# ROAM-Lab-ND/generalized_rbda

Measured on AMD Instinct MI355X. Metric: forward-dynamics evals/sec (batched random states), MIT Humanoid cluster model, higher is better.
Workload: dtype f32; 1 GPU; mit_humanoid.urdf cluster-ABA, 262144 random states per GPU; batch_per_gpu=262144, batch_global=262144, nq=25, nv=24, n_bodies=37, n_clusters=17, parallelism=batch-sharded x1, plan replicated

## Files before the change

generalized_rbda_amd/csrc/capi.cpp:

```cpp
#include <hip/hip_runtime.h>

#include <array>
#include <cassert>
#include <cmath>
#include <cstdio>
#include <cstdlib>
#include <cstring>
#include <map>
#include <memory>
#include <mutex>
#include <string>
#include <vector>

#include "../../include/grbda_hip.h"
#include "../../include/grbda_hip_vjp.h"
#include "../../include/grbda_hip_step_vjp.h"
#include "../../include/grbda_hip_jvp.h"
#include "../../include/grbda_hip_wrench.h"
#include "../../include/grbda_hip_bodies.h"
#include "../../include/grbda_hip_jacobians.h"
#include "../../include/grbda_model_desc.h"
#include "devplan.h"

namespace grbda_hip {
// ... 573 lines not shown
template <class T>
int run_chain(const grbda_plan *p, const DeviceTables &t, const Route &r, const T *q, const T *qd, const T *tau, T *ydd, size_t B, int device,
              void *stream, bool gravity = true, const WrenchList<T> *wrenches = nullptr)
{
    const HostPlan &h = p->host;
    const ChainProgram &cp = h.chain[r.slot];
    const size_t n_tiles = (B + kWave - 1) / kWave;
    const size_t in_rows = static_cast<size_t>(h.nq + 2 * h.nv);
    const hipStream_t hs = static_cast<hipStream_t>(stream);
    ChainDev<T> d = chain_dev<T>(p, t, r.slot);
    if (!gravity)
        for (int i = 0; i < 6; i++) d.a_root[i] = T(0);
    void *scratch = nullptr;
    if (r.path == ROUTE_GEN1) {
        gen1_only(d);
        d.sv_global = 0;
        d.out_lds = -1;
        d.lds_bytes = static_cast<int>(static_cast<size_t>(cp.n_lds) * kWave * sizeof(T));
        const size_t lds_total = gen1_lds_bytes<T>(h, cp);
        const size_t grid = gen1_grid(p, t.n_cu, n_tiles, gen1_waves_per_simd<T>(cp.gens[0].n), lds_total);
        hipError_t e = launch_aba_gen1<T>(d, cp.gens[0].n, cp.gens[0].kind != 0, q, qd, tau, ydd, B, static_cast<int>(grid), lds_total, hs);
        return e == hipSuccess ? GRBDA_OK : hip_err(e, "aba single-cluster launch");
    }
    if (r.path == ROUTE_LM) {
        if (cp.diffs.empty()) d.diffs = nullptr;
        no_gens(d);
        d.n_glb_slots = cp.n_glb + 1;
        d.sv_global = 0;
        const size_t lds_lm = lm_lds_bytes<T>(h, cp);
        d.lds_bytes = static_cast<int>(lds_lm);
        const size_t grid = n_tiles;
        if (int rc = ensure_scratch(p, device, stream, scratch_bytes(grid, static_cast<size_t>(d.n_glb_slots) + in_rows, sizeof(T)), &scratch)) return rc;
        hipError_t e = launch_aba_chain_lm<T>(d, q, qd, tau, ydd, B, static_cast<T *>(scratch), static_cast<int>(grid), lds_lm, hs, r.lm_waves);
        return e == hipSuccess ? GRBDA_OK : hip_err(e, "aba chain launch (latency mode)");
    }
    const int kid = sizeof(T) == 8 ? 1 : 0;
    const size_t waves_per_cu = static_cast<size_t>((sizeof(T) == 8 && !cp.gens.empty()) ? p->opt.waves_per_cu_f64_wide_regs : p->opt.waves_per_cu[kid]);
    const LaunchShape s = launch_shape(t.n_cu, n_tiles, waves_per_cu, static_cast<size_t>(cp.n_lds) * kWave * sizeof(T), h.nq, h.nv, sizeof(T),
                                       static_cast<size_t>(p->opt.lds_bytes_per_wave[kid]), true);
    {
        int n_free_bwd = 0, at_bwd = -1;
        for (size_t i = 0; i < cp.segs.size(); i++)
            if (cp.segs[i].op == SEG_FREE_BWD) { n_free_bwd++; at_bwd = static_cast<int>(i); }
        if (!cp.segs.empty() && cp.segs[0].op == SEG_FREE_FWD && n_free_bwd == 1 && cp.frees[cp.segs[0].first].lds_v >= 0) {
            if (s.stage_all_fits) d.fuse |= 1;
            d.stage_lds_v = cp.frees[cp.segs[0].first].lds_v;
            d.stage_v_index = cp.frees[cp.segs[0].first].v_index;
        }
        if (n_free_bwd == 1 && at_bwd + 1 < static_cast<int>(cp.segs.size()) && cp.segs[at_bwd + 1].op == SEG_FREE_ACC &&
            cp.segs[at_bwd + 1].first == cp.segs[at_bwd].first)
            d.fuse |= 2;
    }
    d.lds_bytes = static_cast<int>(s.lds_bytes);
    if (int rc = ensure_scratch(p, device, stream, scratch_bytes(s.grid, static_cast<size_t>(cp.n_glb) + in_rows, sizeof(T)), &scratch)) return rc;
    hipError_t e = wrenches ? launch_aba_chain_wrench<T>(d, *wrenches, q, qd, tau, ydd, B, static_cast<T *>(scratch), static_cast<int>(s.grid), s.lds_bytes, hs)
                            : launch_aba_chain<T>(d, q, qd, tau, ydd, B, static_cast<T *>(scratch), static_cast<int>(s.grid), s.lds_bytes, hs);
    return e == hipSuccess ? GRBDA_OK : hip_err(e, "aba chain launch");
}

template <class T>
int run_rnea_chain(const grbda_plan *p, const DeviceTables &t, const Route &r, const T *q, const T *qd, const T *ydd, T *tau, size_t B, int device,
                   void *stream, bool gravity = true, const WrenchList<T> *wrenches = nullptr)
{
    const HostPlan &h = p->host;
    const RneaChainProgram &rp = h.rchain[r.slot];
    const size_t n_tiles = (B + kWave - 1) / kWave;
    const size_t in_rows = static_cast<size_t>(h.nq + 2 * h.nv);
    const hipStream_t hs = static_cast<hipStream_t>(stream);
    RneaChainDev<T> d = rnea_chain_dev<T>(p, t, r.slot);
    if (!gravity)
        for (int i = 0; i < 6; i++) d.a_root[i] = T(0);
    void *scratch = nullptr;
    if (r.path == ROUTE_LM) {
        if (rp.diffs.empty()) d.diffs = nullptr;
        no_gens(d);
        d.n_glb_slots = 0;
        const size_t lds_bytes = lm_lds_bytes<T>(h, rp);
        d.lds_bytes = static_cast<int>(lds_bytes);
        const size_t grid = n_tiles;
        if (int rc = ensure_scratch(p, device, stream, scratch_bytes(grid, in_rows, sizeof(T)), &scratch)) return rc;
        hipError_t e = launch_rnea_chain_lm<T>(d, q, qd, ydd, tau, B, static_cast<T *>(scratch), static_cast<int>(grid), lds_bytes, hs, r.lm_waves);
        return e == hipSuccess ? GRBDA_OK : hip_err(e, "rnea chain launch (latency mode)");
    }
    if (r.path == ROUTE_GEN1) {
        gen1_only(d);
        d.lds_bytes = static_cast<int>(static_cast<size_t>(rp.n_lds) * kWave * sizeof(T));
        const size_t lds_total = gen1_lds_bytes<T>(h, rp);
        const size_t grid = gen1_grid(p, t.n_cu, n_tiles, rnea_gen1_waves_per_simd<T>(rp.gens[0].n), lds_total);
        hipError_t e = launch_rnea_gen1<T>(d, rp.gens[0].n, rp.gens[0].kind != 0, q, qd, ydd, tau, B, static_cast<int>(grid), lds_total, hs);
        return e == hipSuccess ? GRBDA_OK : hip_err(e, "rnea single-cluster launch");
    }
    const bool wide = r.slot == SLOT_F32_WIDE;
    const int kid = sizeof(T) == 8 ? 1 : 0;
    const LaunchShape s = launch_shape(t.n_cu, n_tiles, wide ? static_cast<size_t>(16) : static_cast<size_t>(p->opt.waves_per_cu[kid]),
                                       static_cast<size_t>(rp.n_lds) * kWave * sizeof(T), h.nq, h.nv, sizeof(T),
                                       static_cast<size_t>(wide ? p->opt.chain32w_lds_bytes : p->opt.lds_bytes_per_wave[kid]), true);
    d.lds_bytes = static_cast<int>(s.lds_bytes);
    if (int rc = ensure_scratch(p, device, stream, scratch_bytes(s.grid, in_rows + static_cast<size_t>(rp.n_glb), sizeof(T)), &scratch)) return rc;
    const std::vector<ChainFree> &bases = h.chain[r.slot].frees;
    hipError_t e = wrenches ? launch_rnea_chain_wrench<T>(d, *wrenches, bases.empty() ? -1 : bases[0].body, q, qd, ydd, tau, B, static_cast<T *>(scratch),
                                                          static_cast<int>(s.grid), s.lds_bytes, hs)
                            : launch_rnea_chain<T>(d, q, qd, ydd, tau, B, static_cast<T *>(scratch), static_cast<int>(s.grid), s.lds_bytes, hs);
    return e == hipSuccess ? GRBDA_OK : hip_err(e, "rnea chain launch");
}

template <class T>
int projection_run(const grbda_plan *p, bool rnea, const T *q, const T *qd, const T *x, const T *f_ext, T *out, size_t B, int device, void *stream);
// ... 3896 lines not shown
```

generalized_rbda_amd/csrc/chain_kernels.hip:

```cpp
#include <hip/hip_runtime.h>

#include "devplan.h"

#ifndef GRBDA_CHAIN_UNIT
#define GRBDA_CHAIN_UNIT 0
#endif
#define GRBDA_KLDS (GRBDA_CHAIN_UNIT == 3)

namespace grbda_hip {

#include "devmath.h"

template <class T>
struct ChainTables {
    cptr<ChainSeg> segs;
    cptr<ChainLink> links;
    cptr<ChainPair> pairs;
    cptr<ChainFree> frees;
    cptr<ChainDiff> diffs;
    cptr<ChainGen> gens;
    cptr<ChainGenBody> gbodies;
    cptr<int32_t> cints;
    cptr<T> consts;
    int n_segs, nq, nv, ori_repr;
// ... 1461 lines not shown
    P.gens = (cptr<ChainGen>)DP.gens;
    P.gbodies = (cptr<ChainGenBody>)DP.gbodies;
    P.cints = (cptr<int32_t>)DP.cints;
    P.consts = (cptr<T>)DP.consts;
    P.n_segs = 0;
    P.nq = DP.nq;
    P.nv = DP.nv;
    P.ori_repr = DP.ori_repr;
#pragma unroll
    for (int i = 0; i < 6; i++) P.a_root[i] = DP.a_root[i];
    const ChainGen g = load_rec(P.gens);
    gen1_tiles<T, N, LOOP>(DP.lds_bytes, P.nq, q, qd, tau, ydd, B, DP.bad_count, [&](const ChainMemC<T> &M) {
        gen_down<T, N, LOOP>(P, M, g, g.lds_w, true, false);
        gen_up<T, N, LOOP, true>(P, M, g);
    });
}

template <class T, int N, bool LOOP>
static hipError_t launch_gen1(const ChainDev<T> &P, const T *q, const T *qd, const T *tau, T *ydd, size_t B, int grid, size_t lds_bytes,
                              hipStream_t stream)
{
    constexpr int WPS = sizeof(T) == 4 ? (N <= 2 ? 3 : 2) : (N == 1 ? 2 : 1);
    hipLaunchKernelGGL((aba_gen1_kernel<T, N, LOOP, WPS>), dim3(grid), dim3(kWave), lds_bytes, stream, P, q, qd, tau, ydd, B);
    return hipGetLastError();
}
template <class T>
int gen1_waves_per_simd(int n)
{
    return sizeof(T) == 4 ? (n <= 2 ? 3 : 2) : (n == 1 ? 2 : 1);
}
template int gen1_waves_per_simd<float>(int);
template int gen1_waves_per_simd<double>(int);
template <class T>
hipError_t launch_aba_gen1(const ChainDev<T> &P, int n, int implicit, const T *q, const T *qd, const T *tau, T *ydd, size_t B, int grid,
                           size_t lds_bytes, hipStream_t stream)
{
    if (implicit) {
        if (n == 1) return launch_gen1<T, 1, true>(P, q, qd, tau, ydd, B, grid, lds_bytes, stream);
        if (n == 2) return launch_gen1<T, 2, true>(P, q, qd, tau, ydd, B, grid, lds_bytes, stream);
        if (n == 3) return launch_gen1<T, 3, true>(P, q, qd, tau, ydd, B, grid, lds_bytes, stream);
        return launch_gen1<T, 4, true>(P, q, qd, tau, ydd, B, grid, lds_bytes, stream);
    }
    if (n == 1) return launch_gen1<T, 1, false>(P, q, qd, tau, ydd, B, grid, lds_bytes, stream);
    if (n == 2) return launch_gen1<T, 2, false>(P, q, qd, tau, ydd, B, grid, lds_bytes, stream);
    if (n == 3) return launch_gen1<T, 3, false>(P, q, qd, tau, ydd, B, grid, lds_bytes, stream);
    return launch_gen1<T, 4, false>(P, q, qd, tau, ydd, B, grid, lds_bytes, stream);
}
template hipError_t launch_aba_gen1<float>(const ChainDev<float> &, int, int, const float *, const float *, const float *, float *, size_t, int,
                                           size_t, hipStream_t);
template hipError_t launch_aba_gen1<double>(const ChainDev<double> &, int, int, const double *, const double *, const double *, double *,
                                            size_t, int, size_t, hipStream_t);
#endif

template <class T, int WPS, int MODE>
__global__ __launch_bounds__(kWave, WPS) void aba_chain_kernel(ChainDev<T> DP, const T *__restrict__ q, const T *__restrict__ qd,
                                                             const T *__restrict__ tau, T *__restrict__ ydd, size_t B,
                                                             T *__restrict__ scratch)
{
    constexpr bool DIFF = MODE == 1 || MODE == 2, GEN = MODE == 2, INREG = MODE == kModeInReg;
    ChainTables<T> P;
    P.segs = (cptr<ChainSeg>)DP.segs;
    P.links = (cptr<ChainLink>)DP.links;
    P.pairs = (cptr<ChainPair>)DP.pairs;
    P.frees = (cptr<ChainFree>)DP.frees;
    P.diffs = DIFF ? (cptr<ChainDiff>)DP.diffs : nullptr;
    P.gens = GEN ? (cptr<ChainGen>)DP.gens : nullptr;
    P.gbodies = GEN ? (cptr<ChainGenBody>)DP.gbodies : nullptr;
    P.cints = DIFF ? (cptr<int32_t>)DP.cints : nullptr;
    P.consts = (cptr<T>)DP.consts;
    P.n_segs = DP.n_segs;
    P.nq = DP.nq;
    P.nv = DP.nv;
    P.ori_repr = DP.ori_repr;
#pragma unroll
    for (int i = 0; i < 6; i++) P.a_root[i] = DP.a_root[i];
    const int lane = threadIdx.x;
    T *slab = scratch + (size_t)blockIdx.x * (size_t)(DP.n_glb_slots + P.nq + 2 * P.nv) * kWave;
    std::conditional_t<INREG, ChainMemR<T>, ChainMem<T>> M;
    M.lane = lane;
    M.lane_b = (unsigned)lane * (unsigned)sizeof(T);
    M.gmul = 1;
    M.amask = ~0;
    M.glb_u = slab + (size_t)(P.nq + 2 * P.nv) * kWave;
    M.in_q_u = slab;
    M.in_qd_u = slab + (size_t)P.nq * kWave;
    M.in_x_u = slab + (size_t)(P.nq + P.nv) * kWave;
    M.out_u = slab + (size_t)(P.nq + P.nv) * kWave;
    M.set_out(DP.out_lds);
    M.bad = 0;

    const size_t n_tiles = (B + kWave - 1) / kWave;
    for (size_t tile = blockIdx.x; tile < n_tiles; tile += gridDim.x) {
        const size_t left = B - tile * kWave;
        const int rows_valid = left < (size_t)kWave ? (int)left : kWave;
        if constexpr (INREG) stage_inputs_reg<kInRegCols>(q, qd, tau, tile, rows_valid, P.nq, P.nv, M.rq, M.rqd, M.rx, lane, DP.lds_bytes);
        else stage_inputs(q, qd, tau, tile, rows_valid, P.nq, P.nv, slab, lane, DP.lds_bytes);
        if (DP.fuse & 1) {
            const T *mine = reinterpret_cast<const T *>(grbda_smem) + (kWave * P.nq + lane * P.nv + DP.stage_v_index);
            T v[6];
#pragma unroll
            for (int j = 0; j < 6; j++) v[j] = mine[j];
            wave_lds_fence();
            M.lds_st(DP.stage_lds_v, v);
        }
        for (int s = 0; s < P.n_segs; s++) {
            const ChainSeg sg = load_rec(P.segs + s);
            switch (sg.op) {
                case SEG_RUN_FWD:
                    if (DP.sv_global) run_fwd<T, true>(P, M, sg);
                    else run_fwd_c(P, M, sg);
                    break;
                case SEG_RUN_BWD: {
                    if (DP.sv_global) run_bwd<T, false, true>(P, M, sg);
                    else if (sg.rot_kind == 1) run_bwd<T, false, false, 1>(P, M, sg);
                    else run_bwd<T, false, false>(P, M, sg);
                    break;
                }
                case SEG_RUN_ACC:
                    run_acc_c(P, M, sg);
                    break;
                case SEG_PAIR_ACC: pair_acc(P, M, load_rec(P.pairs + sg.first)); break;
                case SEG_FREE_FWD:
                    if (!((DP.fuse & 1) && s == 0)) free_fwd(P, M, load_rec(P.frees + sg.first));
                    break;
                case SEG_FREE_BWD: free_bwd<T, false>(P, M, load_rec(P.frees + sg.first), (DP.fuse & 2) != 0); break;
                case SEG_DIFF_FWD:
                    if constexpr (DIFF) diff_fwd(P, M, load_rec(P.diffs + sg.first));
                    break;
                case SEG_DIFF_BWD:
                    if constexpr (DIFF) diff_bwd<T, false>(P, M, load_rec(P.diffs + sg.first));
                    break;
                case SEG_DIFF_ACC:
                    if constexpr (DIFF) diff_acc(P, M, load_rec(P.diffs + sg.first));
                    break;
                case SEG_GEN_FWD:
                    if constexpr (GEN) gen_segment<T, 0>(P, M, load_rec(P.gens + sg.first));
                    break;
                case SEG_GEN_BWD:
                    if constexpr (GEN) gen_segment<T, 1>(P, M, load_rec(P.gens + sg.first));
                    break;
                case SEG_GEN_ACC:
                    if constexpr (GEN) gen_segment<T, 2>(P, M, load_rec(P.gens + sg.first));
                    break;
                default:
                    if (!(DP.fuse & 2)) free_acc(P, M, load_rec(P.frees + sg.first));
                    break;
            }
        }
        if (M.out_row >= 0) write_outputs_lds<T>(M.out_row, ydd, tile, rows_valid, P.nv, lane);
        else write_outputs(slab + (size_t)(P.nq + P.nv) * kWave, ydd, tile, rows_valid, P.nv, lane);
        M.flush_bad(DP.bad_count, rows_valid);
    }
}


template <class T, int NW, bool DIFF = false>
__global__ __launch_bounds__(NW * kWave) __attribute__((amdgpu_waves_per_eu(2, 2)))
void aba_chain_lm_kernel(ChainDev<T> DP, const T *__restrict__ q, const T *__restrict__ qd, const T *__restrict__ tau,
                         T *__restrict__ ydd, size_t B, T *__restrict__ scratch)
{
    ChainTables<T> P;
    P.segs = (cptr<ChainSeg>)DP.segs;
    P.links = (cptr<ChainLink>)DP.links;
    P.pairs = (cptr<ChainPair>)DP.pairs;
    P.frees = (cptr<ChainFree>)DP.frees;
    P.diffs = DIFF ? (cptr<ChainDiff>)DP.diffs : nullptr;
    P.gens = nullptr;
    P.gbodies = nullptr;
    P.cints = DIFF ? (cptr<int32_t>)DP.cints : nullptr;
    P.consts = (cptr<T>)DP.consts;
    P.n_segs = DP.n_segs;
    P.nq = DP.nq;
    P.nv = DP.nv;
    P.ori_repr = DP.ori_repr;
#pragma unroll
    for (int i = 0; i < 6; i++) P.a_root[i] = DP.a_root[i];
    const int wave = __builtin_amdgcn_readfirstlane((int)(threadIdx.x >> 6)), lane = threadIdx.x & 63;
    T *slab = scratch + (size_t)blockIdx.x * (size_t)(DP.n_glb_slots + P.nq + 2 * P.nv) * kWave;
    unsigned long long *lm_bad = reinterpret_cast<unsigned long long *>(slab + (size_t)(DP.n_glb_slots - 1 + P.nq + 2 * P.nv) * kWave);
    ChainMem<T> M;
    M.bad = 0;
    M.lane = lane;
    M.lane_b = (unsigned)lane * (unsigned)sizeof(T);
    M.gmul = 1;
    M.amask = ~0;
    M.glb_u = slab + (size_t)(P.nq + 2 * P.nv) * kWave;
    M.in_q_u = slab;
    M.in_qd_u = slab + (size_t)P.nq * kWave;
    M.in_x_u = slab + (size_t)(P.nq + P.nv) * kWave;
    M.out_u = slab + (size_t)(P.nq + P.nv) * kWave;
    M.set_out(DP.out_lds);
    const unsigned bq = (unsigned)(kWave * P.nq) * (unsigned)sizeof(T), bv = (unsigned)(kWave * P.nv) * (unsigned)sizeof(T);

    const size_t n_tiles = (B + kWave - 1) / kWave;
    for (size_t tile = blockIdx.x; tile < n_tiles; tile += gridDim.x) {
        const size_t left = B - tile * kWave;
        const int rows_valid = left < (size_t)kWave ? (int)left : kWave;
        if (wave == 0) {
            stage_issue(q, tile, rows_valid, P.nq, 0u, lane);
            asm volatile("s_waitcnt vmcnt(0)" ::: "memory");
            wave_lds_fence();
            stage_transpose(P.nq, 0u, slab, lane);
        } else if (NW == 2) {
// ... 464 lines not shown
#pragma unroll
                    for (int i = 0; i < 6; i++)
#pragma unroll
                        for (int j = 0; j < 6; j++) acc[6 * i + j] += a[i] * b[j];
                }
                if (live) {
#pragma unroll
                    for (int i = 0; i < 6; i++)
#pragma unroll
                        for (int j = 0; j < 6; j++) {
                            Ls[(size_t)(6 * e1 + i) * (6 * m) + 6 * e2 + j] = acc[6 * i + j];
                            Ls[(size_t)(6 * e2 + j) * (6 * m) + 6 * e1 + i] = acc[6 * i + j];
                        }
                }
            }
        asm volatile("s_waitcnt vmcnt(0)" ::: "memory");
    }
}

template <class T>
hipError_t launch_osim_chain(const ChainDev<T> &P, const OsimArgs<T> &A, const T *q, const T *zeros, T *Linv, T *J, size_t B,
                             T *scratch, int grid, size_t lds_bytes, hipStream_t stream)
{
    hipLaunchKernelGGL((osim_chain_kernel<T>), dim3(grid), dim3(kWave), lds_bytes, stream, P, A, q, zeros, Linv, J, B, scratch);
    return hipGetLastError();
}
#if GRBDA_CHAIN_UNIT == 0
template hipError_t launch_osim_chain<float>(const ChainDev<float> &, const OsimArgs<float> &, const float *, const float *, float *,
                                             float *, size_t, float *, int, size_t, hipStream_t);
template hipError_t launch_osim_chain<double>(const ChainDev<double> &, const OsimArgs<double> &, const double *, const double *,
                                              double *, double *, size_t, double *, int, size_t, hipStream_t);
#endif

hipError_t launch_aba_chain_diff_f64(const ChainDev<double> &P, const double *q, const double *qd, const double *tau, double *ydd, size_t B,
                                     double *scratch, int grid, size_t lds_bytes, hipStream_t stream);
template <class T>
hipError_t launch_aba_chain_gen(const ChainDev<T> &P, const T *q, const T *qd, const T *tau, T *ydd, size_t B, T *scratch, int grid,
                                size_t lds_bytes, hipStream_t stream);
template <class T>
hipError_t launch_aba_chain(const ChainDev<T> &P, const T *q, const T *qd, const T *tau, T *ydd, size_t B, T *scratch, int grid,
                            size_t lds_bytes, hipStream_t stream)
{
    if (P.n_gens > 0) return launch_aba_chain_gen<T>(P, q, qd, tau, ydd, B, scratch, grid, lds_bytes, stream);
    if (P.n_diffs > 0) {
        if constexpr (sizeof(T) == 8) {
            return launch_aba_chain_diff_f64(P, q, qd, tau, ydd, B, scratch, grid, lds_bytes, stream);
        } else {
            hipLaunchKernelGGL((aba_chain_kernel<T, 2, 1>), dim3(grid), dim3(kWave), lds_bytes, stream, P, q, qd, tau, ydd, B, scratch);
            return hipGetLastError();
        }
    }
    if constexpr (sizeof(T) == 4) {
        if (chain_inputs_in_registers(sizeof(T), P.n_gens, P.n_diffs, P.sv_global, P.nq, P.nv)) {
            hipLaunchKernelGGL((aba_chain_kernel<T, 2, kModeInReg>), dim3(grid), dim3(kWave), lds_bytes, stream, P, q, qd, tau, ydd, B, scratch);
            return hipGetLastError();
        }
    }
    hipLaunchKernelGGL((aba_chain_kernel<T, 2, 0>), dim3(grid), dim3(kWave), lds_bytes, stream, P, q, qd, tau, ydd, B, scratch);
    return hipGetLastError();
}
#if GRBDA_CHAIN_UNIT == 0
template hipError_t launch_aba_chain<float>(const ChainDev<float> &, const float *, const float *, const float *, float *, size_t,
                                            float *, int, size_t, hipStream_t);
template hipError_t launch_aba_chain<double>(const ChainDev<double> &, const double *, const double *, const double *, double *,
                                             size_t, double *, int, size_t, hipStream_t);
#elif GRBDA_CHAIN_UNIT == 1
hipError_t launch_aba_chain_diff_f64(const ChainDev<double> &P, const double *q, const double *qd, const double *tau, double *ydd, size_t B,
                                     double *scratch, int grid, size_t lds_bytes, hipStream_t stream)
{
    hipLaunchKernelGGL((aba_chain_kernel<double, 2, 1>), dim3(grid), dim3(kWave), lds_bytes, stream, P, q, qd, tau, ydd, B, scratch);
    return hipGetLastError();
}
#elif GRBDA_CHAIN_UNIT == 2
template <class T>
hipError_t launch_aba_chain_gen(const ChainDev<T> &P, const T *q, const T *qd, const T *tau, T *ydd, size_t B, T *scratch, int grid,
                                size_t lds_bytes, hipStream_t stream)
{
    if constexpr (sizeof(T) == 8)
        hipLaunchKernelGGL((aba_chain_kernel<T, 1, 2>), dim3(grid), dim3(kWave), lds_bytes, stream, P, q, qd, tau, ydd, B, scratch);
    else
        hipLaunchKernelGGL((aba_chain_kernel<T, 2, 2>), dim3(grid), dim3(kWave), lds_bytes, stream, P, q, qd, tau, ydd, B, scratch);
    return hipGetLastError();
}
template hipError_t launch_aba_chain_gen<float>(const ChainDev<float> &, const float *, const float *, const float *, float *, size_t,
                                                float *, int, size_t, hipStream_t);
template hipError_t launch_aba_chain_gen<double>(const ChainDev<double> &, const double *, const double *, const double *, double *,
                                                 size_t, double *, int, size_t, hipStream_t);
#elif GRBDA_CHAIN_UNIT == 4
template <class T>
__device__ __forceinline__ void wrench_setup(ChainMemW<T> &M, const WrenchList<T> &W)
{
#pragma unroll
    for (int i = 0; i < kMaxWrenches; i++) M.wbody[i] = W.body[i];
    M.wcanon = W.canon;
}
template <class T>
__device__ __forceinline__ void wrench_tile(ChainMemW<T> &M, const WrenchList<T> &W, size_t tile, size_t B)
{
    const size_t st = tile * kWave + (size_t)M.lane;
    M.wl = W.w + (st < B ? st : B - 1) * (size_t)(W.n * 6);
}
template <class T>
__global__ __launch_bounds__(kWave, 2) void aba_chain_wrench_kernel(ChainDev<T> DP, WrenchList<T> W, const T *__restrict__ q,
                                                                   const T *__restrict__ qd, const T *__restrict__ tau, T *__restrict__ ydd,
                                                                   size_t B, T *__restrict__ scratch)
{
    ChainTables<T> P;
// ... 814 lines not shown
        const size_t left = B - tile * kWave;
        const int rows_valid = left < (size_t)kWave ? (int)left : kWave;
        wrench_tile(M, W, tile, B);
        stage_inputs(q, qd, ydd, tile, rows_valid, P.nq, P.nv, slab, lane, DP.lds_bytes);
        for (int s = 0; s < P.n_segs; s++) {
            const RneaSeg sg = load_rec(P.segs + s);
            switch (sg.op) {
                case RSEG_RUN_FWD: rnea_run_fwd<T, GLB>(P, M, sg); break;
                case RSEG_RUN_BWD: rnea_run_bwd<T, GLB>(P, M, sg); break;
                case RSEG_PAIR: rnea_pair<T, GLB>(P, M, load_rec(P.pairs + sg.first)); break;
                case RSEG_FREE_FWD: rnea_free_fwd(P, M, load_rec(P.frees + sg.first), base_body); break;
                case RSEG_FREE_BWD: rnea_free_bwd(P, M, load_rec(P.frees + sg.first)); break;
                default: break;
            }
        }
        write_outputs(slab + (size_t)(P.nq + P.nv) * kWave, tau, tile, rows_valid, P.nv, lane);
    }
}
template <class T>
hipError_t launch_rnea_chain_wrench(const RneaChainDev<T> &P, const WrenchList<T> &W, int base_body, const T *q, const T *qd, const T *ydd, T *tau,
                                    size_t B, T *scratch, int grid, size_t lds_bytes, hipStream_t stream)
{
    if (P.n_gens > 0 || P.n_diffs > 0 || W.n < 1 || W.n > kMaxWrenches) return hipErrorInvalidValue;
    if (P.n_glb_slots > 0)
        hipLaunchKernelGGL((rnea_chain_wrench_kernel<T, true>), dim3(grid), dim3(kWave), lds_bytes, stream, P, W, base_body, q, qd, ydd, tau, B, scratch);
    else
        hipLaunchKernelGGL((rnea_chain_wrench_kernel<T, false>), dim3(grid), dim3(kWave), lds_bytes, stream, P, W, base_body, q, qd, ydd, tau, B, scratch);
    return hipGetLastError();
}
template hipError_t launch_rnea_chain_wrench<float>(const RneaChainDev<float> &, const WrenchList<float> &, int, const float *, const float *,
                                                    const float *, float *, size_t, float *, int, size_t, hipStream_t);
template hipError_t launch_rnea_chain_wrench<double>(const RneaChainDev<double> &, const WrenchList<double> &, int, const double *, const double *,
                                                     const double *, double *, size_t, double *, int, size_t, hipStream_t);
#endif


static hipError_t set_max_dynamic_lds(const void *const *kernels, int n)
{
    for (int i = 0; i < n; i++) {
        const hipError_t e = hipFuncSetAttribute(kernels[i], hipFuncAttributeMaxDynamicSharedMemorySize, 160 * 1024);
        if (e != hipSuccess) return e;
    }
    return hipSuccess;
}
hipError_t set_max_dynamic_lds_chain_unit1();
hipError_t set_max_dynamic_lds_chain_unit2();
hipError_t set_max_dynamic_lds_chain_unit3();
#if GRBDA_CHAIN_UNIT == 0
hipError_t set_max_dynamic_lds_chain()
{
    const void *const kernels[] = {
        reinterpret_cast<const void *>(&aba_chain_kernel<float, 2, 0>), reinterpret_cast<const void *>(&aba_chain_kernel<float, 2, 1>),
        reinterpret_cast<const void *>(&aba_chain_kernel<float, 2, kModeInReg>),
        reinterpret_cast<const void *>(&aba_chain_kernel<double, 2, 0>),
        reinterpret_cast<const void *>(&rnea_chain_kernel<float, 0, false>), reinterpret_cast<const void *>(&rnea_chain_kernel<float, 1, false>),
        reinterpret_cast<const void *>(&rnea_chain_kernel<double, 0, false>), reinterpret_cast<const void *>(&rnea_chain_kernel<double, 1, false>),
        reinterpret_cast<const void *>(&rnea_chain_kernel<float, 0, true>), reinterpret_cast<const void *>(&rnea_chain_kernel<float, 1, true>),
        reinterpret_cast<const void *>(&rnea_chain_kernel<double, 0, true>), reinterpret_cast<const void *>(&rnea_chain_kernel<double, 1, true>),
        reinterpret_cast<const void *>(&osim_chain_kernel<float>), reinterpret_cast<const void *>(&osim_chain_kernel<double>)};
    const hipError_t e = set_max_dynamic_lds(kernels, static_cast<int>(sizeof(kernels) / sizeof(kernels[0])));
    if (e != hipSuccess) return e;
    const hipError_t e1 = set_max_dynamic_lds_chain_unit1();
    if (e1 != hipSuccess) return e1;
    const hipError_t e2 = set_max_dynamic_lds_chain_unit2();
    return e2 != hipSuccess ? e2 : set_max_dynamic_lds_chain_unit3();
}
#elif GRBDA_CHAIN_UNIT == 1
hipError_t set_max_dynamic_lds_chain_unit1()
{
    const void *const kernels[] = {reinterpret_cast<const void *>(&aba_chain_kernel<double, 2, 1>),
                                   reinterpret_cast<const void *>(&aba_chain_lm_kernel<double, 2>)};
    return set_max_dynamic_lds(kernels, 2);
}
#elif GRBDA_CHAIN_UNIT == 3
hipError_t set_max_dynamic_lds_chain_unit3()
{
    const void *const kernels[] = {reinterpret_cast<const void *>(&aba_chain_lm_kernel<float, 2>), reinterpret_cast<const void *>(&aba_chain_lm_kernel<float, 4>),
                                   reinterpret_cast<const void *>(&aba_chain_lm_kernel<float, 2, true>), reinterpret_cast<const void *>(&aba_chain_lm_kernel<float, 4, true>),
                                   reinterpret_cast<const void *>(&aba_chain_lm_kernel<double, 4>),
                                   reinterpret_cast<const void *>(&rnea_chain_lm_kernel<float, 2>), reinterpret_cast<const void *>(&rnea_chain_lm_kernel<float, 4>),
                                   reinterpret_cast<const void *>(&rnea_chain_lm_kernel<double, 2>), reinterpret_cast<const void *>(&rnea_chain_lm_kernel<double, 4>),
                                   reinterpret_cast<const void *>(&rnea_chain_lm_kernel<float, 2, true>), reinterpret_cast<const void *>(&rnea_chain_lm_kernel<float, 4, true>)};
    return set_max_dynamic_lds(kernels, 11);
}
#elif GRBDA_CHAIN_UNIT == 4
hipError_t set_max_dynamic_lds_chain_wrench()
{
    const void *const kernels[] = {reinterpret_cast<const void *>(&aba_chain_wrench_kernel<float>), reinterpret_cast<const void *>(&aba_chain_wrench_kernel<double>),
                                   reinterpret_cast<const void *>(&rnea_chain_wrench_kernel<float, false>), reinterpret_cast<const void *>(&rnea_chain_wrench_kernel<float, true>),
                                   reinterpret_cast<const void *>(&rnea_chain_wrench_kernel<double, false>), reinterpret_cast<const void *>(&rnea_chain_wrench_kernel<double, true>)};
    return set_max_dynamic_lds(kernels, 6);
}
#else
hipError_t set_max_dynamic_lds_chain_unit2()
{
    const void *const kernels[] = {reinterpret_cast<const void *>(&aba_chain_kernel<float, 2, 2>),
                                   reinterpret_cast<const void *>(&aba_chain_kernel<double, 2, 2>),
                                   reinterpret_cast<const void *>(&rnea_chain_kernel<float, 2, false>),
                                   reinterpret_cast<const void *>(&rnea_chain_kernel<float, 2, true>),
                                   reinterpret_cast<const void *>(&rnea_chain_kernel<double, 2, false>),
                                   reinterpret_cast<const void *>(&rnea_chain_kernel<double, 2, true>)};
    return set_max_dynamic_lds(kernels, 6);
}
#endif

}
// ... 1 lines not shown
```

generalized_rbda_amd/csrc/devmath.h:

```cpp
#pragma once

template <class U>
using cptr = const U __attribute__((address_space(4))) *;

template <class U>
__device__ __forceinline__ U load_rec(cptr<U> p)
{
    static_assert(sizeof(U) % 4 == 0, "plan records are arrays of int32");
    U out;
    cptr<int32_t> src = (cptr<int32_t>)p;
    int32_t *dst = reinterpret_cast<int32_t *>(&out);
#pragma unroll
    for (int i = 0; i < (int)(sizeof(U) / 4); i++) dst[i] = src[i];
    return out;
}

extern __shared__ __attribute__((aligned(16))) unsigned char grbda_smem[];

__host__ __device__ constexpr int sidx(int i, int j)
{
    return i <= j ? (i * 6 - i * (i - 1) / 2 + (j - i)) : (j * 6 - j * (j - 1) / 2 + (i - j));
}

template <class T>
// ... 349 lines not shown
    const unsigned bq = (unsigned)(kWave * nq) * (unsigned)sizeof(T), bv = (unsigned)(kWave * nv) * (unsigned)sizeof(T);
    if ((int)(bq + 2 * bv) <= lds_bytes) {
        stage_issue(q, tile, rows_valid, nq, 0u, lane);
        stage_issue(qd, tile, rows_valid, nv, bq, lane);
        stage_issue(x, tile, rows_valid, nv, bq + bv, lane);
        asm volatile("s_waitcnt vmcnt(0)" ::: "memory");
        wave_lds_fence();
        stage_transpose(nq, 0u, slab, lane);
        stage_transpose(nv, bq, slab + (size_t)nq * kWave, lane);
        stage_transpose(nv, bq + bv, slab + (size_t)(nq + nv) * kWave, lane);
        wave_lds_fence();
    } else {
        stage_issue(q, tile, rows_valid, nq, 0u, lane);
        asm volatile("s_waitcnt vmcnt(0)" ::: "memory");
        wave_lds_fence();
        stage_transpose(nq, 0u, slab, lane);
        wave_lds_fence();
        stage_issue(qd, tile, rows_valid, nv, 0u, lane);
        asm volatile("s_waitcnt vmcnt(0)" ::: "memory");
        wave_lds_fence();
        stage_transpose(nv, 0u, slab + (size_t)nq * kWave, lane);
        wave_lds_fence();
        stage_issue(x, tile, rows_valid, nv, 0u, lane);
        asm volatile("s_waitcnt vmcnt(0)" ::: "memory");
        wave_lds_fence();
        stage_transpose(nv, 0u, slab + (size_t)(nq + nv) * kWave, lane);
        wave_lds_fence();
    }
}

template <class T, int N, class ROW>
__device__ __forceinline__ void stage_row_regs(int ncols, unsigned lds_byte_off, ROW &r, int lane)
{
    const T *stage = reinterpret_cast<const T *>(grbda_smem + lds_byte_off);
    constexpr int V = 16 / (int)sizeof(T);
    static_assert(N % V == 0, "whole 16-byte reads");
    if ((ncols % V) == 0 && (lds_byte_off % 16u) == 0) {
        struct alignas(16) Vec { T v[V]; };
        const Vec *rows = reinterpret_cast<const Vec *>(stage + lane * ncols);
#pragma unroll
        for (int c = 0; c < N; c += V) {
            if (c < ncols) {
                const Vec x = rows[c / V];
#pragma unroll
                for (int k = 0; k < V; k++) r[c + k] = x.v[k];
            }
        }
        return;
    }
#pragma unroll
    for (int c = 0; c < N; c++)
        if (c < ncols) r[c] = stage[lane * ncols + c];
}
template <int N, class T, class ROW>
__device__ __forceinline__ void stage_inputs_reg(const T *__restrict__ q, const T *__restrict__ qd, const T *__restrict__ x, size_t tile,
                                                 int rows_valid, int nq, int nv, ROW &rq, ROW &rqd, ROW &rx, int lane, int lds_bytes)
{
    const unsigned bq = (unsigned)(kWave * nq) * (unsigned)sizeof(T), bv = (unsigned)(kWave * nv) * (unsigned)sizeof(T);
    if ((int)(bq + 2 * bv) <= lds_bytes) {
        stage_issue(q, tile, rows_valid, nq, 0u, lane);
        stage_issue(qd, tile, rows_valid, nv, bq, lane);
        stage_issue(x, tile, rows_valid, nv, bq + bv, lane);
        asm volatile("s_waitcnt vmcnt(0)" ::: "memory");
        wave_lds_fence();
        stage_row_regs<T, N>(nq, 0u, rq, lane);
        stage_row_regs<T, N>(nv, bq, rqd, lane);
        stage_row_regs<T, N>(nv, bq + bv, rx, lane);
        wave_lds_fence();
    } else {
        stage_issue(q, tile, rows_valid, nq, 0u, lane);
        asm volatile("s_waitcnt vmcnt(0)" ::: "memory");
        wave_lds_fence();
        stage_row_regs<T, N>(nq, 0u, rq, lane);
        wave_lds_fence();
        stage_issue(qd, tile, rows_valid, nv, 0u, lane);
        asm volatile("s_waitcnt vmcnt(0)" ::: "memory");
        wave_lds_fence();
        stage_row_regs<T, N>(nv, 0u, rqd, lane);
        wave_lds_fence();
        stage_issue(x, tile, rows_valid, nv, 0u, lane);
        asm volatile("s_waitcnt vmcnt(0)" ::: "memory");
        wave_lds_fence();
        stage_row_regs<T, N>(nv, 0u, rx, lane);
        wave_lds_fence();
    }
}

template <class T>
__device__ __forceinline__ void write_outputs(const T *rows, T *__restrict__ out, size_t tile, int rows_valid, int nv,
                                              int lane)
{
    asm volatile("s_waitcnt vmcnt(0) lgkmcnt(0)" ::: "memory");
    T *stage = reinterpret_cast<T *>(grbda_smem);
    constexpr int V = 16 / (int)sizeof(T);
    if ((nv % V) == 0) {
        struct alignas(16) Vec { T v[V]; };
        Vec *mine = reinterpret_cast<Vec *>(stage + lane * nv);
        for (int c = 0; c < nv; c += V) {
            Vec x;
#pragma unroll
            for (int k = 0; k < V; k++) x.v[k] = rows[(size_t)(c + k) * kWave + lane];
            mine[c / V] = x;
        }
    } else {
        for (int c = 0; c < nv; c++) stage[lane * nv + c] = rows[(size_t)c * kWave + lane];
    }
    wave_lds_fence();
    T *dst = out + tile * (size_t)kWave * (size_t)nv;
    const int total = rows_valid * nv;
    for (int i = 0; i < nv; i++) {
        const int j = i * kWave + lane;
        if (j < total) dst[j] = stage[j];
    }
    wave_lds_fence();
}

template <class T>
__device__ __forceinline__ void write_outputs_lds(int out_row, T *__restrict__ out, size_t tile, int rows_valid, int nv, int lane)
{
    asm volatile("s_waitcnt lgkmcnt(0)" ::: "memory");
    const T *rows = reinterpret_cast<const T *>(grbda_smem) + out_row * kWave;
    T *stage = reinterpret_cast<T *>(grbda_smem) + (out_row >= nv ? 0 : (out_row + nv) * kWave);
    constexpr int V = 16 / (int)sizeof(T);
    if ((nv % V) == 0) {
        struct alignas(16) Vec { T v[V]; };
        Vec *mine = reinterpret_cast<Vec *>(stage + lane * nv);
        for (int c = 0; c < nv; c += V) {
            Vec x;
#pragma unroll
            for (int k = 0; k < V; k++) x.v[k] = rows[(c + k) * kWave + lane];
            mine[c / V] = x;
        }
    } else {
        for (int c = 0; c < nv; c++) stage[lane * nv + c] = rows[c * kWave + lane];
    }
    wave_lds_fence();
    T *dst = out + tile * (size_t)kWave * (size_t)nv;
// ... 164 lines not shown
```

generalized_rbda_amd/csrc/devplan.h:

```cpp
#pragma once
#include <cstdlib>
#include <hip/hip_runtime.h>

#include "plan.h"
#include "walk.h"

namespace grbda_hip {

inline size_t lds_workgroups_per_cu(size_t lds_bytes)
{
    if (lds_bytes == 0) return 32;
    constexpr size_t granule = 1280;
    return (160u * 1024u) / ((lds_bytes + granule - 1) / granule * granule);
}


template <class T>
struct DevPlan {
    const Step *steps;
    int n_steps;
    const ClusterRec *clusters;
    const BodyRec *bodies;
    const T *consts;
    const int32_t *cints;
// ... 10 lines not shown
    T a_root[6];
};

template <class T>
hipError_t launch_aba(const DevPlan<T> &P, const T *q, const T *qd, const T *tau, T *ydd, size_t B, T *scratch,
                      int grid, size_t lds_bytes, hipStream_t stream, bool two_waves_per_simd);
template <class T>
hipError_t launch_rnea(const DevPlan<T> &P, const T *q, const T *qd, const T *ydd, T *tau, size_t B, T *scratch,
                       int grid, size_t lds_bytes, hipStream_t stream);
template <class T>
hipError_t launch_project(const DevPlan<T> &P, int n_clusters, T *q, int32_t *ok, size_t B, int max_iter, T tol,
                          T *scratch, int grid, size_t lds_bytes, hipStream_t stream);
constexpr int kStateFlagWords = 4;
struct StateFlags {
    uint64_t pos[kStateFlagWords], vel[kStateFlagWords];
};
template <class T>
hipError_t launch_state(const DevPlan<T> &P, int n_clusters, const StateFlags &F, const T *q_in, const T *qd_in, int in_nq, int in_nv,
                        T *q_out, T *qd_out, int32_t *status, T *gmax, size_t B, T tol, T *scratch, int grid, size_t lds_bytes,
                        hipStream_t stream);
template <class T>
hipError_t launch_spanning(const DevPlan<T> &P, int n_clusters, int n_span, const T *q, const T *qd, const T *ydd,
                           T *qd_span, T *qdd_span, size_t B, T *scratch, int grid, size_t lds_bytes,
                           hipStream_t stream);
constexpr int kIntegrateLocalRows = kMaxClusterBodies;
template <class T>
hipError_t launch_integrate(const DevPlan<T> &P, int n_clusters, const T *q, const T *qd, const T *ydd, T dt, T *q_next, T *qd_next,
                            int32_t *ok, int ok_and, size_t B, int max_iter, T tol, T *scratch, int grid, size_t lds_bytes, hipStream_t stream);
template <class T>
hipError_t launch_poses(const DevPlan<T> &P, int n_clusters, const T *q, T *Xa, size_t B, int grid, hipStream_t stream);
template <class T>
hipError_t launch_twists(const DevPlan<T> &P, int n_clusters, int n_span, const T *q, const T *qd_span, const T *qdd_span, T *V, size_t B,
                         int grid, hipStream_t stream);
hipError_t set_max_dynamic_lds();

template <class T>
struct ChainDev {
    const ChainSeg *segs;
    const ChainLink *links;
    const ChainPair *pairs;
    const ChainFree *frees;
    const ChainDiff *diffs;
    int n_diffs;
    const ChainGen *gens;
    const ChainGenBody *gbodies;
    int n_gens;
    const int32_t *cints;
    const T *consts;
    int n_segs;
    int nq, nv;
    int n_glb_slots;
    int lds_bytes;
    int ori_repr;
    int debug;
    int sv_global;
    int out_lds;
    int fuse, stage_lds_v, stage_v_index;
    unsigned long long *bad_count;
    T a_root[6];
};
constexpr int kInRegCols = 32;
constexpr int kModeInReg = 3;
inline bool chain_inputs_in_registers(size_t elem, int n_gens, int n_diffs, int sv_global, int nq, int nv)
{
    return elem == 4 && n_gens == 0 && n_diffs == 0 && !sv_global && nq <= kInRegCols && nv <= kInRegCols;
}
template <class T>
hipError_t launch_aba_chain(const ChainDev<T> &P, const T *q, const T *qd, const T *tau, T *ydd, size_t B, T *scratch, int grid,
                            size_t lds_bytes, hipStream_t stream);
template <class T>
hipError_t launch_aba_chain_lm(const ChainDev<T> &P, const T *q, const T *qd, const T *tau, T *ydd, size_t B, T *scratch, int grid,
                               size_t lds_bytes, hipStream_t stream, int n_waves);
hipError_t set_max_dynamic_lds_chain();
template <class T>
hipError_t launch_aba_gen1(const ChainDev<T> &P, int n, int implicit, const T *q, const T *qd, const T *tau, T *ydd, size_t B, int grid,
                           size_t lds_bytes, hipStream_t stream);
template <class T>
int gen1_waves_per_simd(int n);

template <class T>
struct RneaChainDev {
    const RneaSeg *segs;
    const RneaLink *links;
    const RneaPair *pairs;
    const RneaFree *frees;
    const RneaDiff *diffs;
    int n_diffs;
    const ChainGen *gens;
    const ChainGenBody *gbodies;
    int n_gens;
    const int32_t *cints;
    const T *consts;
    int n_segs;
    int nq, nv;
    int n_glb_slots;
    int lds_bytes;
    int ori_repr;
    T a_root[6];
};
template <class T>
hipError_t launch_rnea_chain(const RneaChainDev<T> &P, const T *q, const T *qd, const T *ydd, T *tau, size_t B, T *scratch, int grid,
                             size_t lds_bytes, hipStream_t stream);
template <class T>
hipError_t launch_rnea_chain_lm(const RneaChainDev<T> &P, const T *q, const T *qd, const T *ydd, T *tau, size_t B, T *scratch, int grid, size_t lds_bytes,
                                hipStream_t stream, int n_waves);

constexpr int kMaxWrenches = 16;
template <class T>
struct WrenchList {
    int n;
    int body[kMaxWrenches];
    unsigned canon;
    const T *w;
};
template <class T>
hipError_t launch_aba_chain_wrench(const ChainDev<T> &P, const WrenchList<T> &W, const T *q, const T *qd, const T *tau, T *ydd, size_t B, T *scratch,
                                   int grid, size_t lds_bytes, hipStream_t stream);
template <class T>
// ... 228 lines not shown
```

Measured before the change: 2.270 billion evals/s.

## Load aligned input rows directly into registers, bypassing LDS staging

For the in-register f32 chain ABA kernel, qd and tau (and q when aligned) are now loaded straight from global memory into per-lane register vectors with 16-byte loads. Before, they were staged through LDS with fences. The fused free-body velocity seed now reads from registers instead of LDS. The per-block scratch slab is also shrunk to drop the input rows when inputs live in registers. The aim is to cut LDS round trips and wait barriers at each tile start. The cost is uncoalesced row-strided global loads and more template instantiations. With nq=25, q is not 16-byte divisible, so q still goes through LDS.

```diff
diff --git a/generalized_rbda_amd/csrc/capi.cpp b/generalized_rbda_amd/csrc/capi.cpp
--- a/generalized_rbda_amd/csrc/capi.cpp
+++ b/generalized_rbda_amd/csrc/capi.cpp
@@ -649,7 +649,10 @@
             d.fuse |= 2;
     }
     d.lds_bytes = static_cast<int>(s.lds_bytes);
-    if (int rc = ensure_scratch(p, device, stream, scratch_bytes(s.grid, static_cast<size_t>(cp.n_glb) + in_rows, sizeof(T)), &scratch)) return rc;
+    const bool inreg = !wrenches && chain_inputs_in_registers(sizeof(T), d.n_gens, d.n_diffs, d.sv_global, d.nq, d.nv);
+    if (inreg) d.direct_in = chain_direct_inputs(sizeof(T), d.nq, d.nv, q, qd, tau);
+    const size_t slab_rows = static_cast<size_t>(chain_slab_rows(inreg, d.nq, d.nv, d.n_glb_slots, d.out_lds).total);
+    if (int rc = ensure_scratch(p, device, stream, scratch_bytes(s.grid, slab_rows, sizeof(T)), &scratch)) return rc;
     hipError_t e = wrenches ? launch_aba_chain_wrench<T>(d, *wrenches, q, qd, tau, ydd, B, static_cast<T *>(scratch), static_cast<int>(s.grid), s.lds_bytes, hs)
                             : launch_aba_chain<T>(d, q, qd, tau, ydd, B, static_cast<T *>(scratch), static_cast<int>(s.grid), s.lds_bytes, hs);
     return e == hipSuccess ? GRBDA_OK : hip_err(e, "aba chain launch");
diff --git a/generalized_rbda_amd/csrc/chain_kernels.hip b/generalized_rbda_amd/csrc/chain_kernels.hip
--- a/generalized_rbda_amd/csrc/chain_kernels.hip
+++ b/generalized_rbda_amd/csrc/chain_kernels.hip
@@ -1537,12 +1537,13 @@
                                             size_t, int, size_t, hipStream_t);
 #endif
 
-template <class T, int WPS, int MODE>
+template <class T, int WPS, int MODE, int DIRECT = 0>
 __global__ __launch_bounds__(kWave, WPS) void aba_chain_kernel(ChainDev<T> DP, const T *__restrict__ q, const T *__restrict__ qd,
                                                              const T *__restrict__ tau, T *__restrict__ ydd, size_t B,
                                                              T *__restrict__ scratch)
 {
     constexpr bool DIFF = MODE == 1 || MODE == 2, GEN = MODE == 2, INREG = MODE == kModeInReg;
+    static_assert(INREG || DIRECT == 0, "direct row loads fill the register vectors of kModeInReg");
     ChainTables<T> P;
     P.segs = (cptr<ChainSeg>)DP.segs;
     P.links = (cptr<ChainLink>)DP.links;
@@ -1560,17 +1561,18 @@
 #pragma unroll
     for (int i = 0; i < 6; i++) P.a_root[i] = DP.a_root[i];
     const int lane = threadIdx.x;
-    T *slab = scratch + (size_t)blockIdx.x * (size_t)(DP.n_glb_slots + P.nq + 2 * P.nv) * kWave;
+    const ChainSlabRows rows = chain_slab_rows(INREG, P.nq, P.nv, DP.n_glb_slots, DP.out_lds);
+    T *slab = scratch + (size_t)blockIdx.x * (size_t)rows.total * kWave;
     std::conditional_t<INREG, ChainMemR<T>, ChainMem<T>> M;
     M.lane = lane;
     M.lane_b = (unsigned)lane * (unsigned)sizeof(T);
     M.gmul = 1;
     M.amask = ~0;
-    M.glb_u = slab + (size_t)(P.nq + 2 * P.nv) * kWave;
+    M.glb_u = slab + (size_t)rows.glb * kWave;
     M.in_q_u = slab;
     M.in_qd_u = slab + (size_t)P.nq * kWave;
     M.in_x_u = slab + (size_t)(P.nq + P.nv) * kWave;
-    M.out_u = slab + (size_t)(P.nq + P.nv) * kWave;
+    M.out_u = slab + (size_t)rows.out * kWave;
     M.set_out(DP.out_lds);
     M.bad = 0;
 
@@ -1578,14 +1580,21 @@
     for (size_t tile = blockIdx.x; tile < n_tiles; tile += gridDim.x) {
         const size_t left = B - tile * kWave;
         const int rows_valid = left < (size_t)kWave ? (int)left : kWave;
-        if constexpr (INREG) stage_inputs_reg<kInRegCols>(q, qd, tau, tile, rows_valid, P.nq, P.nv, M.rq, M.rqd, M.rx, lane, DP.lds_bytes);
+        if constexpr (INREG)
+            stage_inputs_reg<kInRegCols, (DIRECT & kDirectQ) != 0, (DIRECT & kDirectQd) != 0, (DIRECT & kDirectX) != 0>(
+                q, qd, tau, tile, rows_valid, P.nq, P.nv, M.rq, M.rqd, M.rx, lane, DP.lds_bytes);
         else stage_inputs(q, qd, tau, tile, rows_valid, P.nq, P.nv, slab, lane, DP.lds_bytes);
         if (DP.fuse & 1) {
-            const T *mine = reinterpret_cast<const T *>(grbda_smem) + (kWave * P.nq + lane * P.nv + DP.stage_v_index);
             T v[6];
-#pragma unroll
-            for (int j = 0; j < 6; j++) v[j] = mine[j];
-            wave_lds_fence();
+            if constexpr ((DIRECT & kDirectQd) != 0) {
+#pragma unroll
+                for (int j = 0; j < 6; j++) v[j] = M.rqd[DP.stage_v_index + j];
+            } else {
+                const T *mine = reinterpret_cast<const T *>(grbda_smem) + (kWave * P.nq + lane * P.nv + DP.stage_v_index);
+#pragma unroll
+                for (int j = 0; j < 6; j++) v[j] = mine[j];
+                wave_lds_fence();
+            }
             M.lds_st(DP.stage_lds_v, v);
         }
         for (int s = 0; s < P.n_segs; s++) {
@@ -1633,7 +1642,7 @@
             }
         }
         if (M.out_row >= 0) write_outputs_lds<T>(M.out_row, ydd, tile, rows_valid, P.nv, lane);
-        else write_outputs(slab + (size_t)(P.nq + P.nv) * kWave, ydd, tile, rows_valid, P.nv, lane);
+        else write_outputs(slab + (size_t)rows.out * kWave, ydd, tile, rows_valid, P.nv, lane);
         M.flush_bad(DP.bad_count, rows_valid);
     }
 }
@@ -2204,7 +2213,14 @@
     }
     if constexpr (sizeof(T) == 4) {
         if (chain_inputs_in_registers(sizeof(T), P.n_gens, P.n_diffs, P.sv_global, P.nq, P.nv)) {
-            hipLaunchKernelGGL((aba_chain_kernel<T, 2, kModeInReg>), dim3(grid), dim3(kWave), lds_bytes, stream, P, q, qd, tau, ydd, B, scratch);
+            if (P.direct_in == (kDirectQ | kDirectQd | kDirectX))
+                hipLaunchKernelGGL((aba_chain_kernel<T, 2, kModeInReg, kDirectQ | kDirectQd | kDirectX>), dim3(grid), dim3(kWave), lds_bytes, stream, P, q, qd,
+                                   tau, ydd, B, scratch);
+            else if (P.direct_in == (kDirectQd | kDirectX))
+                hipLaunchKernelGGL((aba_chain_kernel<T, 2, kModeInReg, kDirectQd | kDirectX>), dim3(grid), dim3(kWave), lds_bytes, stream, P, q, qd, tau,
+                                   ydd, B, scratch);
+            else
+                hipLaunchKernelGGL((aba_chain_kernel<T, 2, kModeInReg>), dim3(grid), dim3(kWave), lds_bytes, stream, P, q, qd, tau, ydd, B, scratch);
             return hipGetLastError();
         }
     }
@@ -3125,6 +3141,8 @@
     const void *const kernels[] = {
         reinterpret_cast<const void *>(&aba_chain_kernel<float, 2, 0>), reinterpret_cast<const void *>(&aba_chain_kernel<float, 2, 1>),
         reinterpret_cast<const void *>(&aba_chain_kernel<float, 2, kModeInReg>),
+        reinterpret_cast<const void *>(&aba_chain_kernel<float, 2, kModeInReg, kDirectQd | kDirectX>),
+        reinterpret_cast<const void *>(&aba_chain_kernel<float, 2, kModeInReg, kDirectQ | kDirectQd | kDirectX>),
         reinterpret_cast<const void *>(&aba_chain_kernel<double, 2, 0>),
         reinterpret_cast<const void *>(&rnea_chain_kernel<float, 0, false>), reinterpret_cast<const void *>(&rnea_chain_kernel<float, 1, false>),
         reinterpret_cast<const void *>(&rnea_chain_kernel<double, 0, false>), reinterpret_cast<const void *>(&rnea_chain_kernel<double, 1, false>),
diff --git a/generalized_rbda_amd/csrc/devmath.h b/generalized_rbda_amd/csrc/devmath.h
--- a/generalized_rbda_amd/csrc/devmath.h
+++ b/generalized_rbda_amd/csrc/devmath.h
@@ -425,37 +425,75 @@
     for (int c = 0; c < N; c++)
         if (c < ncols) r[c] = stage[lane * ncols + c];
 }
-template <int N, class T, class ROW>
+template <class T, int N, class ROW>
+__device__ __forceinline__ void load_row_regs(const T *__restrict__ src, size_t tile, int rows_valid, int ncols, ROW &r, int lane)
+{
+    constexpr int V = 16 / (int)sizeof(T);
+    static_assert(N % V == 0, "whole 16-byte loads");
+    struct alignas(16) Vec { T v[V]; };
+    const int row = lane < rows_valid ? lane : rows_valid - 1;
+    const Vec *mine = reinterpret_cast<const Vec *>(src + (tile * (size_t)kWave + (size_t)row) * (size_t)ncols);
+    const int last = ncols / V - 1;
+#pragma unroll
+    for (int c = 0; c < N; c += V) {
+        const Vec x = mine[c / V < last ? c / V : last];
+#pragma unroll
+        for (int k = 0; k < V; k++) r[c + k] = x.v[k];
+    }
+}
+template <int K>
+__device__ __forceinline__ void wait_all_but_youngest()
+{
+    static_assert(K >= 0 && K < 64, "six bits of vmcnt");
+    asm volatile("s_waitcnt vmcnt(%0)" ::"n"(K) : "memory");
+}
+template <int N, bool DQ, bool DQD, bool DX, class T, class ROW>
 __device__ __forceinline__ void stage_inputs_reg(const T *__restrict__ q, const T *__restrict__ qd, const T *__restrict__ x, size_t tile,
                                                  int rows_valid, int nq, int nv, ROW &rq, ROW &rqd, ROW &rx, int lane, int lds_bytes)
 {
+    constexpr int V = 16 / (int)sizeof(T), kDirectLoads = ((DQ ? 1 : 0) + (DQD ? 1 : 0) + (DX ? 1 : 0)) * (N / V);
     const unsigned bq = (unsigned)(kWave * nq) * (unsigned)sizeof(T), bv = (unsigned)(kWave * nv) * (unsigned)sizeof(T);
     if ((int)(bq + 2 * bv) <= lds_bytes) {
-        stage_issue(q, tile, rows_valid, nq, 0u, lane);
-        stage_issue(qd, tile, rows_valid, nv, bq, lane);
-        stage_issue(x, tile, rows_valid, nv, bq + bv, lane);
-        asm volatile("s_waitcnt vmcnt(0)" ::: "memory");
-        wave_lds_fence();
-        stage_row_regs<T, N>(nq, 0u, rq, lane);
-        stage_row_regs<T, N>(nv, bq, rqd, lane);
-        stage_row_regs<T, N>(nv, bq + bv, rx, lane);
+        if constexpr (!DQ) stage_issue(q, tile, rows_valid, nq, 0u, lane);
+        if constexpr (!DQD) stage_issue(qd, tile, rows_valid, nv, bq, lane);
+        if constexpr (!DX) stage_issue(x, tile, rows_valid, nv, bq + bv, lane);
+        if constexpr (kDirectLoads > 0) asm volatile("" ::: "memory");
+        if constexpr (DQ) load_row_regs<T, N>(q, tile, rows_valid, nq, rq, lane);
+        if constexpr (DQD) load_row_regs<T, N>(qd, tile, rows_valid, nv, rqd, lane);
+        if constexpr (DQD && DX) asm volatile("" ::: "memory");
+        if constexpr (DX) load_row_regs<T, N>(x, tile, rows_valid, nv, rx, lane);
+        if constexpr (DQ && DQD && DX) return;
+        wait_all_but_youngest<kDirectLoads>();
+        wave_lds_fence();
+        if constexpr (!DQ) stage_row_regs<T, N>(nq, 0u, rq, lane);
+        if constexpr (!DQD) stage_row_regs<T, N>(nv, bq, rqd, lane);
+        if constexpr (!DX) stage_row_regs<T, N>(nv, bq + bv, rx, lane);
         wave_lds_fence();
     } else {
-        stage_issue(q, tile, rows_valid, nq, 0u, lane);
-        asm volatile("s_waitcnt vmcnt(0)" ::: "memory");
-        wave_lds_fence();
-        stage_row_regs<T, N>(nq, 0u, rq, lane);
-        wave_lds_fence();
-        stage_issue(qd, tile, rows_valid, nv, 0u, lane);
-        asm volatile("s_waitcnt vmcnt(0)" ::: "memory");
-        wave_lds_fence();
-        stage_row_regs<T, N>(nv, 0u, rqd, lane);
-        wave_lds_fence();
-        stage_issue(x, tile, rows_valid, nv, 0u, lane);
-        asm volatile("s_waitcnt vmcnt(0)" ::: "memory");
-        wave_lds_fence();
-        stage_row_regs<T, N>(nv, 0u, rx, lane);
-        wave_lds_fence();
+        if constexpr (DQ) load_row_regs<T, N>(q, tile, rows_valid, nq, rq, lane);
+        if constexpr (DQD) load_row_regs<T, N>(qd, tile, rows_valid, nv, rqd, lane);
+        if constexpr (DX) load_row_regs<T, N>(x, tile, rows_valid, nv, rx, lane);
+        if constexpr (!DQ) {
+            stage_issue(q, tile, rows_valid, nq, 0u, lane);
+            asm volatile("s_waitcnt vmcnt(0)" ::: "memory");
+            wave_lds_fence();
+            stage_row_regs<T, N>(nq, 0u, rq, lane);
+            wave_lds_fence();
+        }
+        if constexpr (!DQD) {
+            stage_issue(qd, tile, rows_valid, nv, 0u, lane);
+            asm volatile("s_waitcnt vmcnt(0)" ::: "memory");
+            wave_lds_fence();
+            stage_row_regs<T, N>(nv, 0u, rqd, lane);
+            wave_lds_fence();
+        }
+        if constexpr (!DX) {
+            stage_issue(x, tile, rows_valid, nv, 0u, lane);
+            asm volatile("s_waitcnt vmcnt(0)" ::: "memory");
+            wave_lds_fence();
+            stage_row_regs<T, N>(nv, 0u, rx, lane);
+            wave_lds_fence();
+        }
     }
 }
 
diff --git a/generalized_rbda_amd/csrc/devplan.h b/generalized_rbda_amd/csrc/devplan.h
--- a/generalized_rbda_amd/csrc/devplan.h
+++ b/generalized_rbda_amd/csrc/devplan.h
@@ -86,7 +86,7 @@
     int n_glb_slots;
     int lds_bytes;
     int ori_repr;
-    int debug;
+    int direct_in;
     int sv_global;
     int out_lds;
     int fuse, stage_lds_v, stage_v_index;
@@ -98,6 +98,25 @@
 inline bool chain_inputs_in_registers(size_t elem, int n_gens, int n_diffs, int sv_global, int nq, int nv)
 {
     return elem == 4 && n_gens == 0 && n_diffs == 0 && !sv_global && nq <= kInRegCols && nv <= kInRegCols;
+}
+constexpr int kDirectQ = 1, kDirectQd = 2, kDirectX = 4;
+inline int chain_direct_inputs(size_t elem, int nq, int nv, const void *q, const void *qd, const void *x)
+{
+    const auto direct = [elem](int ncols, const void *base) {
+        return (static_cast<size_t>(ncols) * elem) % 16 == 0 && reinterpret_cast<uintptr_t>(base) % 16 == 0;
+    };
+    if (!direct(nv, qd) || !direct(nv, x)) return 0;
+    return kDirectQd | kDirectX | (direct(nq, q) ? kDirectQ : 0);
+}
+struct ChainSlabRows {
+    int glb;
+    int out;
+    int total;
+};
+__host__ __device__ inline ChainSlabRows chain_slab_rows(bool in_registers, int nq, int nv, int n_glb_slots, int out_lds)
+{
+    if (!in_registers) return {nq + 2 * nv, nq + nv, nq + 2 * nv + n_glb_slots};
+    return {0, out_lds < 0 ? n_glb_slots : 0, n_glb_slots + (out_lds < 0 ? nv : 0)};
 }
 template <class T>
 hipError_t launch_aba_chain(const ChainDev<T> &P, const T *q, const T *qd, const T *tau, T *ydd, size_t B, T *scratch, int grid,
```

New measurement: 2.322 billion evals/s (median of 6 runs). 2.3% higher.
